# sangminwoo/SVOL

Hardware: AMD Instinct MI355X
Metric: frames/sec (fwd+matcher+bwd), T=32·P=196·d=256 (higher is better)
Workload: dtype bf16

## Files before the change

svol_amd/csrc/common.h:

```cpp
#pragma once
#include <hip/hip_runtime.h>
#include <stdint.h>

#include "../../include/svol_hip.h"

typedef __bf16 bf16_t;
typedef __attribute__((ext_vector_type(8))) __bf16 bf16x8;
typedef __attribute__((ext_vector_type(4))) __bf16 bf16x4;
typedef __attribute__((ext_vector_type(2))) __bf16 bf16x2;
typedef _Float16 f16_t;
typedef __attribute__((ext_vector_type(8))) _Float16 f16x8;
typedef __attribute__((ext_vector_type(4))) _Float16 f16x4;
typedef __attribute__((ext_vector_type(2))) _Float16 f16x2;
typedef __attribute__((ext_vector_type(4))) float f32x4;
typedef __attribute__((ext_vector_type(16))) float f32x16;

#ifdef SVOL_H16_FP16
typedef f16_t h16_t;
typedef f16x8 h16x8;
typedef f16x4 h16x4;
typedef f16x2 h16x2;
#define SVOL_MFMA_16x16x32_H16 __builtin_amdgcn_mfma_f32_16x16x32_f16
#define SVOL_MFMA_32x32x16_H16 __builtin_amdgcn_mfma_f32_32x32x16_f16
#define SVOL_DS_READ_TR16_H16 svol_ds_read_tr16_f16
// ... 93 lines not shown
    DetScratch& operator=(const DetScratch&) = delete;
};
#ifdef __HIPCC__
namespace {
__global__ __launch_bounds__(256) void det_fold_kernel(const float* __restrict__ part, int parts, int64_t pstride, float* __restrict__ dst,
                                                       int64_t n, int64_t bpart, int64_t bdst) {
    const int64_t j = (int64_t)blockIdx.x * 256 + threadIdx.x;
    if (j >= n) return;
    const float* q = part + (int64_t)blockIdx.y * bpart + j;
    float* d = dst + (int64_t)blockIdx.y * bdst + j;
    float acc = *d;
    for (int i = 0; i < parts; ++i) acc += q[(int64_t)i * pstride];
    *d = acc;
}
inline void det_fold(const float* part, int parts, int64_t pstride, float* dst, int64_t n, hipStream_t s, int batches = 1, int64_t bpart = 0,
                     int64_t bdst = 0) {
    if (!dst || n <= 0 || parts <= 0) return;
    hipLaunchKernelGGL(det_fold_kernel, dim3((unsigned)((n + 255) / 256), (unsigned)batches), dim3(256), 0, s, part, parts, pstride, dst, n,
                       bpart, bdst);
}
}
#endif

struct HalfPair { unsigned lo, hi; };
__device__ __forceinline__ HalfPair swap_halves(unsigned x) {
    unsigned y = x;
    asm volatile("" : "+v"(y));
    const auto sw = __builtin_amdgcn_permlane32_swap(x, y, false, false);
    return HalfPair{sw[0], sw[1]};
}

__device__ __forceinline__ float to_f32(float x) { return x; }
__device__ __forceinline__ float to_f32(bf16_t x) { return (float)x; }
__device__ __forceinline__ float to_f32(f16_t x) { return (float)x; }
template <typename T> __device__ __forceinline__ T from_f32(float x);
template <> __device__ __forceinline__ float from_f32<float>(float x) { return x; }
template <> __device__ __forceinline__ bf16_t from_f32<bf16_t>(float x) { return (bf16_t)x; }
template <> __device__ __forceinline__ f16_t from_f32<f16_t>(float x) { return (f16_t)x; }

template <typename T> struct Vec4;
template <> struct Vec4<float> {
    f32x4 v;
    __device__ __forceinline__ void load(const float* p) { v = *reinterpret_cast<const f32x4*>(p); }
    __device__ __forceinline__ void store(float* p) const { *reinterpret_cast<f32x4*>(p) = v; }
    __device__ __forceinline__ float get(int i) const { return v[i]; }
    __device__ __forceinline__ void set(int i, float x) { v[i] = x; }
// ... 113 lines not shown
```

svol_amd/csrc/gate.hip:

```cpp
#include <cstdlib>

#include "common.h"

namespace {

constexpr int GP = 4;
constexpr int GH = 8;
constexpr int GHMAX = 32;

__device__ __forceinline__ void store_head_sums(const float (&part)[GH], float* __restrict__ scores, int b, int l, int L, int H, int lane,
                                                int h0 = 0) {
    const bool b0 = lane & 1, b1 = lane & 2;
    float h4[4], h2[2];
#pragma unroll
    for (int i = 0; i < 4; ++i) {
        const float send = b0 ? part[i] : part[4 + i], keep = b0 ? part[4 + i] : part[i];
        h4[i] = keep + dpp_f32<0xB1>(send);
    }
#pragma unroll
    for (int i = 0; i < 2; ++i) {
        const float send = b1 ? h4[i] : h4[2 + i], keep = b1 ? h4[2 + i] : h4[i];
        h2[i] = keep + dpp_f32<0x4E>(send);
    }
#pragma unroll
    for (int i = 0; i < 2; ++i) {
        float v = h2[i];
        v += dpp_f32<0x124>(v);
        v += dpp_f32<0x128>(v);
        const HalfPair r16 = swap_rows16(__builtin_bit_cast(unsigned, v));
        v = __builtin_bit_cast(float, r16.lo) + __builtin_bit_cast(float, r16.hi);
        const HalfPair r32 = swap_halves(__builtin_bit_cast(unsigned, v));
        h2[i] = __builtin_bit_cast(float, r32.lo) + __builtin_bit_cast(float, r32.hi);
    }
    if (lane < 4) {
        const int hh0 = h0 + 4 * (lane & 1) + 2 * (lane >> 1);
        if (hh0 < H) scores[((int64_t)b * H + hh0) * L + l] = h2[0];
        if (hh0 + 1 < H) scores[((int64_t)b * H + hh0 + 1) * L + l] = h2[1];
    }
}

template <typename T, int NP, bool WIDE = false>
__global__ __launch_bounds__(256) void gate_scores_kernel(const float* __restrict__ x, const T* __restrict__ pos,
                                                          const float* __restrict__ u, float* __restrict__ scores, int L,
                                                          int D, int H, int rpw, int hbase) {
    const int lane = threadIdx.x & 63, wave = threadIdx.x >> 6;
    const int b = blockIdx.y;
    const int l0 = (blockIdx.x * 4 + wave) * rpw;
    const int h0 = WIDE ? hbase : 0;
    float ur[GH][NP][4];
#pragma unroll
    for (int hh = 0; hh < GH; ++hh)
#pragma unroll
        for (int j = 0; j < NP; ++j) {
            const int c = (lane + 64 * j) * 4;
#pragma unroll
            for (int e = 0; e < 4; ++e) ur[hh][j][e] = (h0 + hh < H && c < D) ? u[((int64_t)b * H + h0 + hh) * D + c + e] : 0.f;
        }
    const int lend = min(l0 + rpw, L);
    Vec4<float> xv[NP], nxv[NP];
    Vec4<T> pv[NP], npv[NP];
    auto fetch = [&](int l, Vec4<float> (&xr)[NP], Vec4<T> (&pr)[NP]) {
        const int64_t row = (int64_t)b * L + l;
#pragma unroll
        for (int j = 0; j < NP; ++j) {
            const int c = (lane + 64 * j) * 4;
            if (c < D) {
                xr[j].load(x + row * D + c);
                pr[j].load(pos + row * D + c);
            }
        }
    };
    if (l0 < lend) fetch(l0, xv, pv);
    for (int l = l0; l < lend; ++l) {
        if (l + 1 < lend) fetch(l + 1, nxv, npv);
        float part[GH];
#pragma unroll
        for (int hh = 0; hh < GH; ++hh) part[hh] = 0.f;
#pragma unroll
        for (int j = 0; j < NP; ++j) {
            const int c = (lane + 64 * j) * 4;
            if (c < D) {
#pragma unroll
                for (int e = 0; e < 4; ++e) {
                    const float t = xv[j].get(e) + pv[j].get(e);
#pragma unroll
                    for (int hh = 0; hh < GH; ++hh) part[hh] += t * ur[hh][j][e];
                }
            }
        }
        store_head_sums(part, scores, b, l, L, H, lane, h0);
#pragma unroll
        for (int j = 0; j < NP; ++j) { xv[j] = nxv[j]; pv[j] = npv[j]; }
    }
}

__global__ __launch_bounds__(256) void gate_stats_kernel(const float* __restrict__ scores, float* __restrict__ mx_out,
                                                         float* __restrict__ sm_out, int L) {
    __shared__ float red[4];
    const int bh = blockIdx.x, tid = threadIdx.x, lane = tid & 63, wave = tid >> 6;
    const float* s = scores + (int64_t)bh * L;
    float m = -INFINITY;
    for (int l = tid; l < L; l += 256) m = fmaxf(m, s[l]);
    m = wave_max(m);
    if (lane == 0) red[wave] = m;
    __syncthreads();
    m = fmaxf(fmaxf(red[0], red[1]), fmaxf(red[2], red[3]));
    __syncthreads();
    float acc = 0.f;
    for (int l = tid; l < L; l += 256) acc += __expf(s[l] - m);
    acc = wave_sum(acc);
    if (lane == 0) red[wave] = acc;
    __syncthreads();
    if (tid == 0) {
        mx_out[bh] = m;
        sm_out[bh] = red[0] + red[1] + red[2] + red[3];
    }
// ... 171 lines not shown
        }
    }
    __syncthreads();
    float part[GH];
#pragma unroll
    for (int hh = 0; hh < GH; ++hh) part[hh] = 0.f;
#pragma unroll
    for (int j = 0; j < NP; ++j) {
        const int c = (lane + 64 * j) * 4;
        if (c < D) {
            f32x4 ur[GH];
#pragma unroll
            for (int hh = 0; hh < GH; ++hh) ur[hh] = *reinterpret_cast<const f32x4*>(su + hh * D + c);
#pragma unroll
            for (int e = 0; e < 4; ++e) {
#pragma unroll
                for (int hh = 0; hh < GH; ++hh) part[hh] += tp[j][e] * ur[hh][e];
            }
        }
    }
    store_head_sums(part, scores, b, l, L, H, lane);
}

template <typename T, int NP>
__global__ __launch_bounds__(256) void gate_bwd_ln_kernel(const float* __restrict__ dy32, const T* __restrict__ dy,
                                                          const T* __restrict__ dy2, const float* __restrict__ x,
                                                          const float* __restrict__ a_in,
                                                          const float* __restrict__ gamma, const float* __restrict__ mean,
                                                          const float* __restrict__ rstd, float* __restrict__ dx,
                                                          float* __restrict__ da, float* __restrict__ dgamma,
                                                          float* __restrict__ dbeta, const float* __restrict__ scores,
                                                          const float* __restrict__ mx, const float* __restrict__ sm,
                                                          float* __restrict__ cc, int L, int H, int64_t M, int D, int rpw,
                                                          float* __restrict__ det_cc, float* __restrict__ det_gb) {
    const int lane = threadIdx.x & 63;
    const int64_t r0 = ((int64_t)blockIdx.x * 4 + (threadIdx.x >> 6)) * rpw;
    const int64_t rend = (r0 + rpw < M) ? r0 + rpw : M;
    float dg[NP][4], db[NP][4], gm[NP][4];
    int bcur = r0 < rend ? (int)(r0 / L) : 0, lcur = r0 < rend ? (int)(r0 % L) : 0;
    float cacc = 0.f, mxl = 0.f, isl = 0.f;
    if (lane < H && r0 < rend) { mxl = mx[bcur * H + lane]; isl = 1.f / sm[bcur * H + lane]; }
#pragma unroll
    for (int j = 0; j < NP; ++j) {
        const int c = (lane + 64 * j) * 4;
#pragma unroll
        for (int e = 0; e < 4; ++e) { dg[j][e] = 0.f; db[j][e] = 0.f; gm[j][e] = c < D ? gamma[c + e] : 0.f; }
    }
    struct Row { Vec4<float> p32[NP], xv[NP]; Vec4<T> p[NP], p2[NP]; float mu, rs, a, sc; };
    auto fetch = [&](int64_t row, int b, int l, Row& r) {
#pragma unroll
        for (int j = 0; j < NP; ++j) {
            const int c = (lane + 64 * j) * 4;
            if (c < D) {
                if (dy32) r.p32[j].load(dy32 + row * D + c);
                if (dy) r.p[j].load(dy + row * D + c);
                if (dy2) r.p2[j].load(dy2 + row * D + c);
                r.xv[j].load(x + row * D + c);
            }
        }
        r.mu = mean[row]; r.rs = rstd[row]; r.a = a_in[row];
        r.sc = lane < H ? scores[((int64_t)b * H + lane) * L + l] : 0.f;
    };
    Row cur, nxt;
    if (r0 < rend) fetch(r0, bcur, lcur, cur);
    for (int64_t row = r0; row < rend; ++row) {
        int bn = bcur, ln = lcur + 1;
        if (ln == L) { ln = 0; ++bn; }
        if (row + 1 < rend) fetch(row + 1, bn, ln, nxt);
        const float mu = cur.mu, rs = cur.rs, a = cur.a;
        float g[NP][4], xh[NP][4];
        float s1 = 0.f, s2 = 0.f;
#pragma unroll
        for (int j = 0; j < NP; ++j) {
            const int c = (lane + 64 * j) * 4;
            if (c < D) {
#pragma unroll
                for (int e = 0; e < 4; ++e) {
                    const float d = (dy32 ? cur.p32[j].get(e) : 0.f) + (dy ? cur.p[j].get(e) : 0.f) + (dy2 ? cur.p2[j].get(e) : 0.f);
                    const float hv = (cur.xv[j].get(e) * (1.f + a) - mu) * rs;
                    xh[j][e] = hv;
                    dg[j][e] += d * hv;
                    db[j][e] += d;
                    const float gg = d * gm[j][e];
                    g[j][e] = gg;
                    s1 += gg;
                    s2 += gg * hv;
                }
            }
        }
        s1 = wave_sum(s1) / (float)D;
        s2 = wave_sum(s2) / (float)D;
        float dacc = 0.f;
#pragma unroll
        for (int j = 0; j < NP; ++j) {
            const int c = (lane + 64 * j) * 4;
            if (c < D) {
                Vec4<float> o;
#pragma unroll
                for (int e = 0; e < 4; ++e) {
                    const float ds = rs * (g[j][e] - s1 - xh[j][e] * s2);
                    dacc += ds * cur.xv[j].get(e);
                    o.set(e, ds * (1.f + a));
                }
                o.store(dx + row * D + c);
            }
        }
        dacc = wave_sum(dacc);
        if (lane == 0) da[row] = dacc;
        cacc += __expf(cur.sc - mxl) * isl * dacc;
        if (bn != bcur || row + 1 == rend) {
            if (lane < H) {
                if (det_cc) det_cc[(((int64_t)blockIdx.x * 4 + (threadIdx.x >> 6)) * (M / L) + bcur) * H + lane] = cacc / (float)H;
                else atomicAdd(cc + bcur * H + lane, cacc / (float)H);
                cacc = 0.f;
                if (row + 1 < rend) { mxl = mx[bn * H + lane]; isl = 1.f / sm[bn * H + lane]; }
            }
        }
        bcur = bn;
        lcur = ln;
        cur = nxt;
    }
    __shared__ float red[2][NP * 256];
    const int wave = threadIdx.x >> 6;
    for (int w = 0; w < 4; ++w) {
        if (wave == w) {
#pragma unroll
            for (int j = 0; j < NP; ++j) {
                const int c = (lane + 64 * j) * 4;
                if (c < D) {
#pragma unroll
                    for (int e = 0; e < 4; ++e) {
                        if (w == 0) { red[0][c + e] = dg[j][e]; red[1][c + e] = db[j][e]; }
                        else { red[0][c + e] += dg[j][e]; red[1][c + e] += db[j][e]; }
                    }
                }
            }
        }
        __syncthreads();
    }
    if (det_gb) {
        float* row = det_gb + (int64_t)blockIdx.x * 2 * D;
        for (int c = threadIdx.x; c < D; c += 256) { row[c] = red[0][c]; row[D + c] = red[1][c]; }
        return;
    }
    for (int c = threadIdx.x; c < D; c += 256) {
        atomicAdd(dgamma + c, red[0][c]);
        atomicAdd(dbeta + c, red[1][c]);
    }
}

template <typename T, int NP, bool WIDE = false>
__global__ __launch_bounds__(256) void gate_bwd_apply_kernel(const float* __restrict__ x, const T* __restrict__ pos,
                                                             const float* __restrict__ u, const float* __restrict__ scores,
                                                             const float* __restrict__ mx, const float* __restrict__ sm,
                                                             const float* __restrict__ da, const float* __restrict__ cc,
                                                             float* __restrict__ dx, float* __restrict__ du, int L, int D,
                                                             int H, int rpw, float* __restrict__ det_du, int hbase) {
    const int lane = threadIdx.x & 63, wave = threadIdx.x >> 6;
    const int b = blockIdx.y;
    const int l0 = (blockIdx.x * 4 + wave) * rpw;
    const int h0 = WIDE ? hbase : 0;
    float ur[GH][NP][4], dur[GH][NP][4];
#pragma unroll
    for (int hh = 0; hh < GH; ++hh)
#pragma unroll
        for (int j = 0; j < NP; ++j) {
            const int c = (lane + 64 * j) * 4;
#pragma unroll
            for (int e = 0; e < 4; ++e) {
                ur[hh][j][e] = (h0 + hh < H && c < D) ? u[((int64_t)b * H + h0 + hh) * D + c + e] : 0.f;
                dur[hh][j][e] = 0.f;
            }
        }
    const int lend = min(l0 + rpw, L);
    Vec4<float> xv[NP], dv[NP], nxv[NP], ndv[NP];
    Vec4<T> pv[NP], npv[NP];
    float mxr[GH], isr[GH], ccr[GH], sc[GH], nsc[GH], dar = 0.f, ndar = 0.f;
#pragma unroll
    for (int hh = 0; hh < GH; ++hh) {
        mxr[hh] = h0 + hh < H ? mx[b * H + h0 + hh] : 0.f;
        isr[hh] = h0 + hh < H ? 1.f / sm[b * H + h0 + hh] : 0.f;
        ccr[hh] = h0 + hh < H ? cc[b * H + h0 + hh] : 0.f;
        sc[hh] = nsc[hh] = 0.f;
    }
    auto fetch = [&](int l, Vec4<float> (&xr)[NP], Vec4<T> (&pr)[NP], Vec4<float> (&dr)[NP], float (&sr)[GH], float& dr1) {
        const int64_t row = (int64_t)b * L + l;
#pragma unroll
        for (int j = 0; j < NP; ++j) {
            const int c = (lane + 64 * j) * 4;
            if (c < D) {
                xr[j].load(x + row * D + c);
                pr[j].load(pos + row * D + c);
                dr[j].load(dx + row * D + c);
            }
        }
#pragma unroll
        for (int hh = 0; hh < GH; ++hh)
            if (h0 + hh < H) sr[hh] = scores[((int64_t)b * H + h0 + hh) * L + l];
        dr1 = da[row];
    };
    if (l0 < lend) fetch(l0, xv, pv, dv, sc, dar);
    for (int l = l0; l < lend; ++l) {
        const int64_t row = (int64_t)b * L + l;
        if (l + 1 < lend) fetch(l + 1, nxv, npv, ndv, nsc, ndar);
        float ds[GH];
        const float dal = dar / (float)H;
#pragma unroll
        for (int hh = 0; hh < GH; ++hh) {
            if (h0 + hh < H) {
                const float pp = __expf(sc[hh] - mxr[hh]) * isr[hh];
                ds[hh] = pp * (dal - ccr[hh]);
            } else ds[hh] = 0.f;
        }
#pragma unroll
        for (int j = 0; j < NP; ++j) {
            const int c = (lane + 64 * j) * 4;
            if (c < D) {
#pragma unroll
                for (int e = 0; e < 4; ++e) {
                    const float t = xv[j].get(e) + pv[j].get(e);
                    float add = 0.f;
#pragma unroll
                    for (int hh = 0; hh < GH; ++hh) {
                        add += ds[hh] * ur[hh][j][e];
                        dur[hh][j][e] += ds[hh] * t;
                    }
                    dv[j].set(e, dv[j].get(e) + add);
                }
                dv[j].store(dx + row * D + c);
            }
        }
#pragma unroll
        for (int j = 0; j < NP; ++j) { xv[j] = nxv[j]; pv[j] = npv[j]; dv[j] = ndv[j]; }
#pragma unroll
        for (int hh = 0; hh < GH; ++hh) sc[hh] = nsc[hh];
        dar = ndar;
    }
    __shared__ float red[GH * NP * 256];
    for (int w = 0; w < 4; ++w) {
        if (wave == w) {
#pragma unroll
            for (int hh = 0; hh < GH; ++hh)
#pragma unroll
                for (int j = 0; j < NP; ++j) {
                    const int c = (lane + 64 * j) * 4;
#pragma unroll
                    for (int e = 0; e < 4; ++e) {
                        float* r = red + hh * NP * 256 + c + e;
                        if (w == 0) *r = dur[hh][j][e];
                        else *r += dur[hh][j][e];
                    }
                }
        }
        __syncthreads();
    }
    for (int i = threadIdx.x; i < GH * NP * 256; i += 256) {
        const int hh = i / (NP * 256), c = i % (NP * 256);
        if (h0 + hh < H && c < D) {
            if (det_du) det_du[(((int64_t)b * gridDim.x + blockIdx.x) * H + h0 + hh) * D + c] = red[i];
            else atomicAdd(du + ((int64_t)b * H + h0 + hh) * D + c, red[i]);
// ... 161 lines not shown
}

}

extern "C" {

static int gate_fwd_impl(const float* x32, const void* pos, const float* u, const float* gamma, const float* beta, float* y32,
                         void* y, void* ypos, float* a, float* mean, float* rstd, float* ws, int64_t B, int64_t L, int64_t D, int64_t H,
                         int dtype, void* stream, bool scored) {
    if (!x32 || !pos || !u || !gamma || !beta || (!y && !y32) || !a || !mean || !rstd || !ws) return SVOL_E_INVALID;
    if (!aligned16(gamma) || !aligned16(beta)) return SVOL_E_INVALID;
    if (B <= 0 || L <= 0 || D <= 0 || H <= 0) return SVOL_E_INVALID;
    if (D % 4 || D > GP * 256 || H > (scored ? GH : GHMAX) || B > 65535 || L > (1 << 24)) return SVOL_E_UNSUPPORTED;
    if (!svol_is16(dtype) && dtype != SVOL_F32) return SVOL_E_INVALID;
    hipStream_t s = reinterpret_cast<hipStream_t>(stream);
    const int np_ = D <= 256 ? 1 : (D <= 512 ? 2 : 4);
    float* scores = ws;
    float* mx = ws + B * H * L;
    float* sm = mx + B * H;
    const int rpw = rows_per_wave(L, gate_waves(0) / B + 1);
    dim3 g1((unsigned)((L + 4 * rpw - 1) / (4 * rpw)), (unsigned)B);
    const int64_t M = B * L;
    const unsigned g3 = (unsigned)((M + 3) / 4);
#define SVOL_GATE_SC(TT, N, W, H0) hipLaunchKernelGGL((gate_scores_kernel<TT, N, W>), g1, dim3(256), 0, s, x32, (const TT*)pos, u, scores, (int)L, (int)D, (int)H, rpw, H0)
#define SVOL_GATE_AP(TT, N, W, H0) hipLaunchKernelGGL((gate_apply_kernel<TT, N, W>), dim3(g3), dim3(256), 0, s, x32, (const TT*)pos, scores, mx, sm, gamma, beta, y32, (TT*)y, (TT*)ypos, a, mean, rstd, (int)L, (int)D, (int)H, M)
#define SVOL_GATE_NP(LAUNCH, TT, W, H0)                                                                                     \
    do {                                                                                                                    \
        if (np_ == 1) LAUNCH(TT, 1, W, H0);                                                                                 \
        else if (np_ == 2) LAUNCH(TT, 2, W, H0);                                                                            \
        else LAUNCH(TT, 4, W, H0);                                                                                          \
    } while (0)
#define SVOL_GATE_FWD(TT)                                                                                                   \
    do {                                                                                                                    \
        if (scored) { }                                                                                                      \
        else if (H <= GH) SVOL_GATE_NP(SVOL_GATE_SC, TT, false, 0);                                                         \
        else for (int h0 = 0; h0 < (int)H; h0 += GH) SVOL_GATE_NP(SVOL_GATE_SC, TT, true, h0);                              \
        hipLaunchKernelGGL(gate_stats_kernel, dim3((unsigned)(B * H)), dim3(256), 0, s, scores, mx, sm, (int)L);            \
        if (H <= GH) SVOL_GATE_NP(SVOL_GATE_AP, TT, false, 0);                                                              \
        else SVOL_GATE_NP(SVOL_GATE_AP, TT, true, 0);                                                                       \
    } while (0)
    if (dtype == SVOL_BF16) SVOL_GATE_FWD(bf16_t);
    else if (dtype == SVOL_F16) SVOL_GATE_FWD(f16_t);
    else SVOL_GATE_FWD(float);
#undef SVOL_GATE_FWD
#undef SVOL_GATE_SC
#undef SVOL_GATE_AP
    SVOL_CHECK_LAUNCH();
    return SVOL_OK;
}

int svol_gate_fwd(const float* x32, const void* pos, const float* u, const float* gamma, const float* beta, float* y32,
                  void* y, void* ypos, float* a, float* mean, float* rstd, float* ws, int64_t B, int64_t L, int64_t D, int64_t H,
                  int dtype, void* stream) {
    return gate_fwd_impl(x32, pos, u, gamma, beta, y32, y, ypos, a, mean, rstd, ws, B, L, D, H, dtype, stream, false);
}

int svol_gate_fwd_scored(const float* x32, const void* pos, const float* u, const float* gamma, const float* beta, float* y32,
                         void* y, void* ypos, float* a, float* mean, float* rstd, float* ws, int64_t B, int64_t L, int64_t D,
                         int64_t H, int dtype, void* stream) {
// ... 32 lines not shown
    if (B <= 0 || L <= 0 || D <= 0 || H <= 0) return SVOL_E_INVALID;
    if (D % 4 || D > GP * 256 || H > GHMAX || B > 65535 || L > (1 << 24)) return SVOL_E_UNSUPPORTED;
    if (!svol_is16(dtype) && dtype != SVOL_F32) return SVOL_E_INVALID;
    hipStream_t s = reinterpret_cast<hipStream_t>(stream);
    const int np_ = D <= 256 ? 1 : (D <= 512 ? 2 : 4);
    const float* scores = ws;
    const float* mx = ws + B * H * L;
    const float* sm = mx + B * H;
    float* da = ws2;
    float* cc = ws2 + B * L;
    const int64_t M = B * L;
    const int rpw1 = rows_per_wave(M, gate_waves(1));
    const unsigned g1 = (unsigned)(((M + rpw1 - 1) / rpw1 + 3) / 4);
    const int rpw3 = rows_per_wave(L, gate_waves(2) / B + 1);
    dim3 g3((unsigned)((L + 4 * rpw3 - 1) / (4 * rpw3)), (unsigned)B);
    if (hipMemsetAsync(cc, 0, sizeof(float) * (size_t)(B * H), s) != hipSuccess) return SVOL_E_LAUNCH;
    const bool det_mode = svol_deterministic();
    const size_t n_cc = (size_t)g1 * 4 * (size_t)(B * H), n_gb = (size_t)g1 * 2 * (size_t)D, n_du = (size_t)B * g3.x * (size_t)(H * D);
    DetScratch det(det_mode ? n_cc + n_gb + n_du : 0, s, true);
    if (det_mode && !det.p) return SVOL_E_LAUNCH;
    float* det_cc = det_mode ? det.p : nullptr;
    float* det_gb = det_mode ? det.p + n_cc : nullptr;
    float* det_du = det_mode ? det.p + n_cc + n_gb : nullptr;
#define SVOL_GATE_LN(TT, N, W, H0) hipLaunchKernelGGL((gate_bwd_ln_kernel<TT, N>), dim3(g1), dim3(256), 0, s, dy32, (const TT*)dy, (const TT*)dy2, x32, a, gamma, mean, rstd, dx32, da, dgamma, dbeta, scores, mx, sm, cc, (int)L, (int)H, M, (int)D, rpw1, det_cc, det_gb)
#define SVOL_GATE_BA(TT, N, W, H0) hipLaunchKernelGGL((gate_bwd_apply_kernel<TT, N, W>), g3, dim3(256), 0, s, x32, (const TT*)pos, u, scores, mx, sm, da, cc, dx32, du, (int)L, (int)D, (int)H, rpw3, det_du, H0)
#define SVOL_GATE_BWD(TT)                                                                                                   \
    do {                                                                                                                    \
        SVOL_GATE_NP(SVOL_GATE_LN, TT, false, 0);                                                                           \
        if (det_mode) {                                                                                                     \
            det_fold(det_cc, (int)(g1 * 4), B * H, cc, B * H, s);                                                           \
            det_fold(det_gb, (int)g1, 2 * D, dgamma, D, s);                                                                 \
            det_fold(det_gb + D, (int)g1, 2 * D, dbeta, D, s);                                                              \
        }                                                                                                                   \
        if (H <= GH) SVOL_GATE_NP(SVOL_GATE_BA, TT, false, 0);                                                              \
        else for (int h0 = 0; h0 < (int)H; h0 += GH) SVOL_GATE_NP(SVOL_GATE_BA, TT, true, h0);                              \
    } while (0)
    if (dtype == SVOL_BF16) SVOL_GATE_BWD(bf16_t);
    else if (dtype == SVOL_F16) SVOL_GATE_BWD(f16_t);
    else SVOL_GATE_BWD(float);
#undef SVOL_GATE_BWD
#undef SVOL_GATE_LN
#undef SVOL_GATE_BA
#undef SVOL_GATE_NP
    if (det_mode) det_fold(det_du, (int)g3.x, H * D, du, H * D, s, (int)B, (int64_t)g3.x * H * D, H * D);
    SVOL_CHECK_LAUNCH();
    return SVOL_OK;
}

int svol_gate_vectors_fwd(const float* skch, const float* W_in, const float* b_in, float* q_out, float* u_out, int64_t B, int64_t D,
                          int64_t H, void* stream) {
    if (!skch || !W_in || !b_in || !q_out || !u_out || B <= 0 || D <= 0 || H <= 0) return SVOL_E_INVALID;
    if (D % 4 || D > GP * 256 || H > GHMAX || D % H || B > 65535) return SVOL_E_UNSUPPORTED;
    if (!aligned16(W_in)) return SVOL_E_INVALID;
    hipLaunchKernelGGL(gate_vec_fwd_kernel, dim3((unsigned)H, (unsigned)B), dim3(256), 0, reinterpret_cast<hipStream_t>(stream), skch,
                       W_in, b_in, q_out, u_out, (int)D, (int)H);
    SVOL_CHECK_LAUNCH();
    return SVOL_OK;
}

int svol_gate_vectors_bwd(const float* du, const float* skch, const float* W_in, const float* q, float* dq_ws, float* dskch,
                          float* dW_in, float* db_in, int64_t B, int64_t D, int64_t H, void* stream) {
    if (!du || !skch || !W_in || !q || !dq_ws || !dW_in || !db_in || B <= 0 || D <= 0 || H <= 0) return SVOL_E_INVALID;
    if (D % 4 || D > GP * 256 || H > GHMAX || D % H || B > 65535) return SVOL_E_UNSUPPORTED;
    if (!aligned16(W_in)) return SVOL_E_INVALID;
    hipStream_t s = reinterpret_cast<hipStream_t>(stream);
    hipLaunchKernelGGL(gate_vec_bwd_a_kernel, dim3((unsigned)H, (unsigned)B), dim3(256), 0, s, du, W_in, dq_ws, (int)D, (int)H);
// ... 42 lines not shown
```

svol_amd/csrc/norm.hip:

```cpp
#include "common.h"

namespace {

constexpr int LN_MAX_PASSES = 4;

template <typename T, typename TX, int NP>
__global__ __launch_bounds__(256) void ln_fwd_kernel(const TX* __restrict__ x, const float* __restrict__ gamma,
                                                     const float* __restrict__ beta, float* __restrict__ y32,
                                                     T* __restrict__ y, T* __restrict__ ypos, const T* __restrict__ pos,
                                                     int64_t pos_rows, float* __restrict__ mean, float* __restrict__ rstd,
                                                     int64_t M, int D, float p, float inv_keep, uint64_t seed0,
                                                     const int64_t* __restrict__ soff) {
    const uint64_t seed = seed0 + (soff ? ((uint64_t)soff[0] << 8) : 0ull);
    const int lane = threadIdx.x & 63;
    const int64_t row = (int64_t)blockIdx.x * 4 + (threadIdx.x >> 6);
    if (row >= M) return;
    const TX* xr = x + row * D;
    float v[NP][4];
    float s = 0.f;
    const T* pr = pos ? pos + (row % pos_rows) * D : nullptr;
    Vec4<TX> t[NP];
    Vec4<T> pv[NP];
    Vec4<float> gv[NP], bv[NP];
#pragma unroll
// ... 28 lines not shown
    const float rs = rsqrtf(wave_sum(q) / (float)D + 1e-5f);
    if (lane == 0) { mean[row] = mu; rstd[row] = rs; }
#pragma unroll
    for (int j = 0; j < NP; ++j) {
        const int c = (lane + 64 * j) * 4;
        if (c < D) {
            Vec4<T> o, op;
            Vec4<float> o32;
#pragma unroll
            for (int e = 0; e < 4; ++e) {
                float r = (v[j][e] - mu) * rs * gv[j].get(e) + bv[j].get(e);
                if (p > 0.f) r *= dropout_scale(seed, (uint64_t)row, (uint32_t)(c + e), p, inv_keep);
                o.set(e, r);
                o32.set(e, r);
                if (pr) op.set(e, r + pv[j].get(e));
            }
            if (y32) o32.store(y32 + row * D + c);
            if (y) o.store(y + row * D + c);
            if (ypos) op.store(ypos + row * D + c);
        }
    }
}

template <typename T, typename TX, int NP>
__global__ __launch_bounds__(256) void ln_bwd_kernel(const float* __restrict__ dy32, const T* __restrict__ dy,
                                                     const T* __restrict__ dy2, const TX* __restrict__ x,
                                                     const float* __restrict__ gamma, const float* __restrict__ mean,
                                                     const float* __restrict__ rstd, float* __restrict__ dx32,
                                                     T* __restrict__ dx, float* __restrict__ dgamma,
                                                     float* __restrict__ dbeta, float* __restrict__ dxsum, int64_t M, int D,
                                                     float p, float inv_keep, uint64_t seed0, const int64_t* __restrict__ soff, int rows_per_wave,
                                                     float* __restrict__ det_part) {
    const uint64_t seed = seed0 + (soff ? ((uint64_t)soff[0] << 8) : 0ull);
    const int lane = threadIdx.x & 63;
    const int64_t wave_id = (int64_t)blockIdx.x * 4 + (threadIdx.x >> 6);
    const int64_t r0 = wave_id * rows_per_wave;
    float dg[NP][4], db[NP][4], dxs[NP][4], gm[NP][4];
#pragma unroll
    for (int j = 0; j < NP; ++j) {
        const int c = (lane + 64 * j) * 4;
#pragma unroll
        for (int e = 0; e < 4; ++e) { dg[j][e] = 0.f; db[j][e] = 0.f; dxs[j][e] = 0.f; gm[j][e] = c < D ? gamma[c + e] : 0.f; }
    }
    struct Row { Vec4<float> a32[NP]; Vec4<T> a[NP], b[NP]; Vec4<TX> xv[NP]; float mu, rs; };
    auto fetch = [&](int64_t row, Row& r) {
#pragma unroll
        for (int j = 0; j < NP; ++j) {
            const int c = (lane + 64 * j) * 4;
            if (c < D) {
                if (dy32) r.a32[j].load(dy32 + row * D + c);
                if (dy) r.a[j].load(dy + row * D + c);
                if (dy2) r.b[j].load(dy2 + row * D + c);
                r.xv[j].load(x + row * D + c);
            }
        }
        r.mu = mean[row];
        r.rs = rstd[row];
    };
    const int64_t rend = (r0 + rows_per_wave < M) ? r0 + rows_per_wave : M;
    Row cur, nxt;
    if (r0 < rend) fetch(r0, cur);
    for (int64_t row = r0; row < rend; ++row) {
        if (row + 1 < rend) fetch(row + 1, nxt);
        const float mu = cur.mu, rs = cur.rs;
        float g[NP][4], xh[NP][4];
        float s1 = 0.f, s2 = 0.f;
#pragma unroll
        for (int j = 0; j < NP; ++j) {
            const int c = (lane + 64 * j) * 4;
            if (c < D) {
#pragma unroll
                for (int e = 0; e < 4; ++e) {
                    float d = (dy32 ? cur.a32[j].get(e) : 0.f) + (dy ? cur.a[j].get(e) : 0.f) + (dy2 ? cur.b[j].get(e) : 0.f);
                    if (p > 0.f) d *= dropout_scale(seed, (uint64_t)row, (uint32_t)(c + e), p, inv_keep);
                    const float h = (cur.xv[j].get(e) - mu) * rs;
                    xh[j][e] = h;
                    dg[j][e] += d * h;
                    db[j][e] += d;
                    const float gg = d * gm[j][e];
                    g[j][e] = gg;
                    s1 += gg;
                    s2 += gg * h;
                }
            }
        }
        s1 = wave_sum(s1) / (float)D;
        s2 = wave_sum(s2) / (float)D;
#pragma unroll
        for (int j = 0; j < NP; ++j) {
            const int c = (lane + 64 * j) * 4;
            if (c < D) {
                Vec4<T> o;
                Vec4<float> o32;
#pragma unroll
                for (int e = 0; e < 4; ++e) {
                    const float r = rs * (g[j][e] - s1 - xh[j][e] * s2);
                    dxs[j][e] += r;
                    o.set(e, r);
                    o32.set(e, r);
                }
                if (dx32) o32.store(dx32 + row * D + c);
                if (dx) o.store(dx + row * D + c);
            }
        }
        cur = nxt;
    }
    __shared__ float red[3][NP * 256];
    const int wave = threadIdx.x >> 6;
    for (int w = 0; w < 4; ++w) {
        if (wave == w) {
#pragma unroll
            for (int j = 0; j < NP; ++j) {
                const int c = (lane + 64 * j) * 4;
                if (c < D) {
#pragma unroll
                    for (int e = 0; e < 4; ++e) {
                        if (w == 0) { red[0][c + e] = dg[j][e]; red[1][c + e] = db[j][e]; red[2][c + e] = dxs[j][e]; }
                        else { red[0][c + e] += dg[j][e]; red[1][c + e] += db[j][e]; red[2][c + e] += dxs[j][e]; }
                    }
                }
            }
        }
        __syncthreads();
    }
    if (det_part) {
        float* row = det_part + (int64_t)blockIdx.x * 3 * D;
        for (int c = threadIdx.x; c < D; c += 256) { row[c] = red[0][c]; row[D + c] = red[1][c]; row[2 * D + c] = red[2][c]; }
        return;
    }
// ... 123 lines not shown
    SVOL_CHECK_LAUNCH();
    return SVOL_OK;
}

int svol_layernorm_bwd(const float* dy32, const void* dy, const void* dy2, const void* x, int x_f32, const float* gamma,
                       const float* mean, const float* rstd, float* dx32, void* dx, float* dgamma, float* dbeta,
                       float* dx_colsum, int64_t M, int64_t D, float dropout_p, uint64_t seed, const int64_t* seed_offset_dev,
                       int dtype, void* stream) {
    if ((!dy32 && !dy && !dy2) || !x || !gamma || !mean || !rstd || (!dx && !dx32) || !dgamma || !dbeta || M < 0 || D <= 0)
        return SVOL_E_INVALID;
    if (D % 4 || D > LN_MAX_PASSES * 256) return SVOL_E_UNSUPPORTED;
    if (dropout_p < 0.f || dropout_p >= 1.f) return SVOL_E_INVALID;
    if (!svol_is16(dtype) && dtype != SVOL_F32) return SVOL_E_INVALID;
    if (M == 0) return SVOL_OK;
    const float inv_keep = 1.f / (1.f - dropout_p);
    int64_t rpw = (M + 2047) / 2048;
    if (rpw < 1) rpw = 1;
    const int64_t waves = (M + rpw - 1) / rpw;
    const unsigned grid = (unsigned)((waves + 3) / 4);
    hipStream_t s = reinterpret_cast<hipStream_t>(stream);
    const bool det_mode = svol_deterministic();
    DetScratch det(det_mode ? (size_t)grid * 3 * (size_t)D : 0, s);
    if (det_mode && !det.p) return SVOL_E_LAUNCH;
#define SVOL_LNB(TT, TXX, NPP)                                                                                                      \
    hipLaunchKernelGGL((ln_bwd_kernel<TT, TXX, NPP>), dim3(grid), dim3(256), 0, s, dy32, (const TT*)dy, (const TT*)dy2, (const TXX*)x, \
                       gamma, mean, rstd, dx32, (TT*)dx, dgamma, dbeta, dx_colsum, M, (int)D, dropout_p, inv_keep, seed,              \
                       seed_offset_dev, (int)rpw, det.p)
#define SVOL_LNB_NP(TT, TXX)                  \
    do {                                      \
        if (D <= 256) SVOL_LNB(TT, TXX, 1);   \
        else if (D <= 512) SVOL_LNB(TT, TXX, 2); \
        else SVOL_LNB(TT, TXX, 4);            \
    } while (0)
    if (dtype == SVOL_BF16 && x_f32) SVOL_LNB_NP(bf16_t, float);
    else if (dtype == SVOL_BF16) SVOL_LNB_NP(bf16_t, bf16_t);
    else if (dtype == SVOL_F16 && x_f32) SVOL_LNB_NP(f16_t, float);
    else if (dtype == SVOL_F16) SVOL_LNB_NP(f16_t, f16_t);
    else SVOL_LNB_NP(float, float);
#undef SVOL_LNB_NP
#undef SVOL_LNB
    if (det_mode) {
        det_fold(det.p, (int)grid, 3 * D, dgamma, D, s);
        det_fold(det.p + D, (int)grid, 3 * D, dbeta, D, s);
        det_fold(det.p + 2 * D, (int)grid, 3 * D, dx_colsum, D, s);
    }
    SVOL_CHECK_LAUNCH();
    return SVOL_OK;
}

int svol_dropout_sd(const void* x, void* y, int64_t n, int64_t row_len, float p, uint64_t seed, const int64_t* seed_step_dev, int dtype,
                    void* stream) {
    if (!x || !y || n < 0 || row_len <= 0 || row_len > 0xffffffffll || !(p >= 0.f && p < 1.f)) return SVOL_E_INVALID;
    if (n == 0) return SVOL_OK;
    const float inv = 1.f / (1.f - p);
    int64_t g = (n + 1023) / 1024;
// ... 48 lines not shown
```

Measured before the change: 14980.

## Add templated ring-buffer row prefetch to gate and layernorm backward row loops

Replaces the single next-row double buffer in the gate scores, gate backward LN/apply and layernorm backward kernels with a generic ring of PF prefetched rows. Loads become unconditional by clamping columns and substituting a dummy source for null pointers, which removes branches and keeps more loads in flight. Depth is chosen at runtime from an environment variable and defaults to 2, so by default the pipeline depth matches the old code apart from the branch-free loads and an FMA change. Deeper settings raise register pressure and may reduce occupancy.

```diff
diff --git a/svol_amd/csrc/common.h b/svol_amd/csrc/common.h
--- a/svol_amd/csrc/common.h
+++ b/svol_amd/csrc/common.h
@@ -139,6 +139,42 @@
 }
 #endif
 
+constexpr int ROWLOOP_DEPTH_SHIPPED = 2;
+template <int PF, typename Fetch, typename Body>
+__host__ __device__ __forceinline__ void row_ring(int64_t r0, int64_t rend, Fetch&& fetch, Body&& body) {
+    if (r0 >= rend) return;
+    const int64_t last = rend - 1;
+#pragma unroll
+    for (int s = 0; s < PF; ++s) fetch(r0 + s < last ? r0 + s : last, s);
+    for (int64_t base = r0; base < rend; base += PF) {
+#pragma unroll
+        for (int s = 0; s < PF; ++s) {
+            const int64_t row = base + s;
+            if (row >= rend) return;
+            body(row, s);
+            fetch(row + PF < last ? row + PF : last, s);
+        }
+    }
+}
+__host__ __device__ __forceinline__ int rowloop_col(int c, int D) { return c < D ? c : D - 4; }
+template <typename T> struct RowSrc { const T* p; int64_t ld; };
+template <typename T>
+__host__ __device__ __forceinline__ RowSrc<T> rowloop_src(const T* p, int64_t ld, const float* spare) {
+    return p ? RowSrc<T>{p, ld} : RowSrc<T>{reinterpret_cast<const T*>(spare), 0};
+}
+static inline int svol_rowloop_depth() {
+    static const int depth = [] {
+        const char* e = getenv("SVOL_ROWLOOP_DEPTH");
+        const int v = e ? atoi(e) : ROWLOOP_DEPTH_SHIPPED;
+        return v >= 8 ? 8 : (v >= 4 ? 4 : 2);
+    }();
+    return depth;
+}
+constexpr int rowloop_slots(int depth, int np, int cap = 8) {
+    const int d = depth < cap ? depth : cap;
+    return np == 1 ? d : (np == 2 && d >= 4 && cap >= 8 ? 4 : 2);
+}
+
 struct HalfPair { unsigned lo, hi; };
 __device__ __forceinline__ HalfPair swap_halves(unsigned x) {
     unsigned y = x;
diff --git a/svol_amd/csrc/gate.hip b/svol_amd/csrc/gate.hip
--- a/svol_amd/csrc/gate.hip
+++ b/svol_amd/csrc/gate.hip
@@ -6,6 +6,8 @@
 
 constexpr int GP = 4;
 constexpr int GH = 8;
+constexpr int GATE_AP_SLOTS = 4;
+template <typename T> constexpr int gate_ln_slots() { return sizeof(T) == 4 ? 4 : 8; }
 constexpr int GHMAX = 32;
 
 __device__ __forceinline__ void store_head_sums(const float (&part)[GH], float* __restrict__ scores, int b, int l, int L, int H, int lane,
@@ -39,7 +41,7 @@
     }
 }
 
-template <typename T, int NP, bool WIDE = false>
+template <typename T, int NP, int PF, bool WIDE = false>
 __global__ __launch_bounds__(256) void gate_scores_kernel(const float* __restrict__ x, const T* __restrict__ pos,
                                                           const float* __restrict__ u, float* __restrict__ scores, int L,
                                                           int D, int H, int rpw, int hbase) {
@@ -57,41 +59,38 @@
             for (int e = 0; e < 4; ++e) ur[hh][j][e] = (h0 + hh < H && c < D) ? u[((int64_t)b * H + h0 + hh) * D + c + e] : 0.f;
         }
     const int lend = min(l0 + rpw, L);
-    Vec4<float> xv[NP], nxv[NP];
-    Vec4<T> pv[NP], npv[NP];
-    auto fetch = [&](int l, Vec4<float> (&xr)[NP], Vec4<T> (&pr)[NP]) {
+    struct Row { Vec4<float> xv[NP]; Vec4<T> pv[NP]; };
+    Row ring[PF];
+    auto fetch = [&](int64_t l, int slot) __attribute__((always_inline)) {
+        Row& r = ring[slot];
         const int64_t row = (int64_t)b * L + l;
+#pragma unroll
+        for (int j = 0; j < NP; ++j) {
+            const int c = rowloop_col((lane + 64 * j) * 4, D);
+            r.xv[j].load(x + row * D + c);
+            r.pv[j].load(pos + row * D + c);
+        }
+    };
+    auto body = [&](int64_t l, int slot) __attribute__((always_inline)) {
+        const Row& cur = ring[slot];
+        float part[GH];
+#pragma unroll
+        for (int hh = 0; hh < GH; ++hh) part[hh] = 0.f;
 #pragma unroll
         for (int j = 0; j < NP; ++j) {
             const int c = (lane + 64 * j) * 4;
             if (c < D) {
-                xr[j].load(x + row * D + c);
-                pr[j].load(pos + row * D + c);
-            }
-        }
-    };
-    if (l0 < lend) fetch(l0, xv, pv);
-    for (int l = l0; l < lend; ++l) {
-        if (l + 1 < lend) fetch(l + 1, nxv, npv);
-        float part[GH];
-#pragma unroll
-        for (int hh = 0; hh < GH; ++hh) part[hh] = 0.f;
-#pragma unroll
-        for (int j = 0; j < NP; ++j) {
-            const int c = (lane + 64 * j) * 4;
-            if (c < D) {
 #pragma unroll
                 for (int e = 0; e < 4; ++e) {
-                    const float t = xv[j].get(e) + pv[j].get(e);
+                    const float t = cur.xv[j].get(e) + cur.pv[j].get(e);
 #pragma unroll
                     for (int hh = 0; hh < GH; ++hh) part[hh] += t * ur[hh][j][e];
                 }
             }
         }
-        store_head_sums(part, scores, b, l, L, H, lane, h0);
-#pragma unroll
-        for (int j = 0; j < NP; ++j) { xv[j] = nxv[j]; pv[j] = npv[j]; }
-    }
+        store_head_sums(part, scores, b, (int)l, L, H, lane, h0);
+    };
+    row_ring<PF>(l0, lend, fetch, body);
 }
 
 __global__ __launch_bounds__(256) void gate_stats_kernel(const float* __restrict__ scores, float* __restrict__ mx_out,
@@ -309,7 +308,7 @@
     store_head_sums(part, scores, b, l, L, H, lane);
 }
 
-template <typename T, int NP>
+template <typename T, int NP, int PF>
 __global__ __launch_bounds__(256) void gate_bwd_ln_kernel(const float* __restrict__ dy32, const T* __restrict__ dy,
                                                           const T* __restrict__ dy2, const float* __restrict__ x,
                                                           const float* __restrict__ a_in,
@@ -334,26 +333,34 @@
         for (int e = 0; e < 4; ++e) { dg[j][e] = 0.f; db[j][e] = 0.f; gm[j][e] = c < D ? gamma[c + e] : 0.f; }
     }
     struct Row { Vec4<float> p32[NP], xv[NP]; Vec4<T> p[NP], p2[NP]; float mu, rs, a, sc; };
-    auto fetch = [&](int64_t row, int b, int l, Row& r) {
+    Row ring[PF];
+    int bf = bcur, lf = lcur;
+    int64_t rf = r0;
+    const RowSrc<float> q32 = rowloop_src(dy32, D, gamma);
+    const RowSrc<T> qa = rowloop_src(dy, D, gamma), qb = rowloop_src(dy2, D, gamma);
+    const int hl = lane < H ? lane : H - 1;
+    auto fetch = [&](int64_t row, int slot) __attribute__((always_inline)) {
+        Row& r = ring[slot];
+        lf += row != rf ? 1 : 0;
+        rf = row;
+        const bool wrap = lf == L;
+        lf = wrap ? 0 : lf;
+        bf += wrap ? 1 : 0;
 #pragma unroll
         for (int j = 0; j < NP; ++j) {
-            const int c = (lane + 64 * j) * 4;
-            if (c < D) {
-                if (dy32) r.p32[j].load(dy32 + row * D + c);
-                if (dy) r.p[j].load(dy + row * D + c);
-                if (dy2) r.p2[j].load(dy2 + row * D + c);
-                r.xv[j].load(x + row * D + c);
-            }
+            const int c = rowloop_col((lane + 64 * j) * 4, D);
+            r.p32[j].load(q32.p + row * q32.ld + c);
+            r.p[j].load(qa.p + row * qa.ld + c);
+            r.p2[j].load(qb.p + row * qb.ld + c);
+            r.xv[j].load(x + row * D + c);
         }
         r.mu = mean[row]; r.rs = rstd[row]; r.a = a_in[row];
-        r.sc = lane < H ? scores[((int64_t)b * H + lane) * L + l] : 0.f;
+        r.sc = scores[((int64_t)bf * H + hl) * L + lf];
     };
-    Row cur, nxt;
-    if (r0 < rend) fetch(r0, bcur, lcur, cur);
-    for (int64_t row = r0; row < rend; ++row) {
+    auto body = [&](int64_t row, int slot) __attribute__((always_inline)) {
+        const Row& cur = ring[slot];
         int bn = bcur, ln = lcur + 1;
         if (ln == L) { ln = 0; ++bn; }
-        if (row + 1 < rend) fetch(row + 1, bn, ln, nxt);
         const float mu = cur.mu, rs = cur.rs, a = cur.a;
         float g[NP][4], xh[NP][4];
         float s1 = 0.f, s2 = 0.f;
@@ -366,7 +373,7 @@
                     const float d = (dy32 ? cur.p32[j].get(e) : 0.f) + (dy ? cur.p[j].get(e) : 0.f) + (dy2 ? cur.p2[j].get(e) : 0.f);
                     const float hv = (cur.xv[j].get(e) * (1.f + a) - mu) * rs;
                     xh[j][e] = hv;
-                    dg[j][e] += d * hv;
+                    dg[j][e] = __builtin_fmaf(d, hv, dg[j][e]);
                     db[j][e] += d;
                     const float gg = d * gm[j][e];
                     g[j][e] = gg;
@@ -405,8 +412,8 @@
         }
         bcur = bn;
         lcur = ln;
-        cur = nxt;
-    }
+    };
+    row_ring<PF>(r0, rend, fetch, body);
     __shared__ float red[2][NP * 256];
     const int wave = threadIdx.x >> 6;
     for (int w = 0; w < 4; ++w) {
@@ -436,7 +443,7 @@
     }
 }
 
-template <typename T, int NP, bool WIDE = false>
+template <typename T, int NP, int PF, bool WIDE = false>
 __global__ __launch_bounds__(256) void gate_bwd_apply_kernel(const float* __restrict__ x, const T* __restrict__ pos,
                                                              const float* __restrict__ u, const float* __restrict__ scores,
                                                              const float* __restrict__ mx, const float* __restrict__ sm,
@@ -460,69 +467,61 @@
             }
         }
     const int lend = min(l0 + rpw, L);
-    Vec4<float> xv[NP], dv[NP], nxv[NP], ndv[NP];
-    Vec4<T> pv[NP], npv[NP];
-    float mxr[GH], isr[GH], ccr[GH], sc[GH], nsc[GH], dar = 0.f, ndar = 0.f;
+    float mxr[GH], isr[GH], ccr[GH];
 #pragma unroll
     for (int hh = 0; hh < GH; ++hh) {
         mxr[hh] = h0 + hh < H ? mx[b * H + h0 + hh] : 0.f;
         isr[hh] = h0 + hh < H ? 1.f / sm[b * H + h0 + hh] : 0.f;
         ccr[hh] = h0 + hh < H ? cc[b * H + h0 + hh] : 0.f;
-        sc[hh] = nsc[hh] = 0.f;
-    }
-    auto fetch = [&](int l, Vec4<float> (&xr)[NP], Vec4<T> (&pr)[NP], Vec4<float> (&dr)[NP], float (&sr)[GH], float& dr1) {
+    }
+    struct Row { Vec4<float> xv[NP], dv[NP]; Vec4<T> pv[NP]; float sc[GH], da; };
+    Row ring[PF];
+    auto fetch = [&](int64_t l, int slot) __attribute__((always_inline)) {
+        Row& r = ring[slot];
         const int64_t row = (int64_t)b * L + l;
+#pragma unroll
+        for (int j = 0; j < NP; ++j) {
+            const int c = rowloop_col((lane + 64 * j) * 4, D);
+            r.xv[j].load(x + row * D + c);
+            r.pv[j].load(pos + row * D + c);
+            r.dv[j].load(dx + row * D + c);
+        }
+#pragma unroll
+        for (int hh = 0; hh < GH; ++hh) r.sc[hh] = scores[((int64_t)b * H + min(h0 + hh, H - 1)) * L + l];
+        r.da = da[row];
+    };
+    auto body = [&](int64_t l, int slot) __attribute__((always_inline)) {
+        Row& cur = ring[slot];
+        const int64_t row = (int64_t)b * L + l;
+        float ds[GH];
+        const float dal = cur.da / (float)H;
+#pragma unroll
+        for (int hh = 0; hh < GH; ++hh) {
+            if (h0 + hh < H) {
+                const float pp = __expf(cur.sc[hh] - mxr[hh]) * isr[hh];
+                ds[hh] = pp * (dal - ccr[hh]);
+            } else ds[hh] = 0.f;
+        }
 #pragma unroll
         for (int j = 0; j < NP; ++j) {
             const int c = (lane + 64 * j) * 4;
             if (c < D) {
-                xr[j].load(x + row * D + c);
-                pr[j].load(pos + row * D + c);
-                dr[j].load(dx + row * D + c);
-            }
-        }
-#pragma unroll
-        for (int hh = 0; hh < GH; ++hh)
-            if (h0 + hh < H) sr[hh] = scores[((int64_t)b * H + h0 + hh) * L + l];
-        dr1 = da[row];
-    };
-    if (l0 < lend) fetch(l0, xv, pv, dv, sc, dar);
-    for (int l = l0; l < lend; ++l) {
-        const int64_t row = (int64_t)b * L + l;
-        if (l + 1 < lend) fetch(l + 1, nxv, npv, ndv, nsc, ndar);
-        float ds[GH];
-        const float dal = dar / (float)H;
-#pragma unroll
-        for (int hh = 0; hh < GH; ++hh) {
-            if (h0 + hh < H) {
-                const float pp = __expf(sc[hh] - mxr[hh]) * isr[hh];
-                ds[hh] = pp * (dal - ccr[hh]);
-            } else ds[hh] = 0.f;
-        }
-#pragma unroll
-        for (int j = 0; j < NP; ++j) {
-            const int c = (lane + 64 * j) * 4;
-            if (c < D) {
 #pragma unroll
                 for (int e = 0; e < 4; ++e) {
-                    const float t = xv[j].get(e) + pv[j].get(e);
+                    const float t = cur.xv[j].get(e) + cur.pv[j].get(e);
                     float add = 0.f;
 #pragma unroll
                     for (int hh = 0; hh < GH; ++hh) {
                         add += ds[hh] * ur[hh][j][e];
                         dur[hh][j][e] += ds[hh] * t;
                     }
-                    dv[j].set(e, dv[j].get(e) + add);
+                    cur.dv[j].set(e, cur.dv[j].get(e) + add);
                 }
-                dv[j].store(dx + row * D + c);
-            }
-        }
-#pragma unroll
-        for (int j = 0; j < NP; ++j) { xv[j] = nxv[j]; pv[j] = npv[j]; dv[j] = ndv[j]; }
-#pragma unroll
-        for (int hh = 0; hh < GH; ++hh) sc[hh] = nsc[hh];
-        dar = ndar;
-    }
+                cur.dv[j].store(dx + row * D + c);
+            }
+        }
+    };
+    row_ring<PF>(l0, lend, fetch, body);
     __shared__ float red[GH * NP * 256];
     for (int w = 0; w < 4; ++w) {
         if (wave == w) {
@@ -730,7 +729,7 @@
     dim3 g1((unsigned)((L + 4 * rpw - 1) / (4 * rpw)), (unsigned)B);
     const int64_t M = B * L;
     const unsigned g3 = (unsigned)((M + 3) / 4);
-#define SVOL_GATE_SC(TT, N, W, H0) hipLaunchKernelGGL((gate_scores_kernel<TT, N, W>), g1, dim3(256), 0, s, x32, (const TT*)pos, u, scores, (int)L, (int)D, (int)H, rpw, H0)
+#define SVOL_GATE_SC(TT, N, PFF, W, H0) hipLaunchKernelGGL((gate_scores_kernel<TT, N, PFF, W>), g1, dim3(256), 0, s, x32, (const TT*)pos, u, scores, (int)L, (int)D, (int)H, rpw, H0)
 #define SVOL_GATE_AP(TT, N, W, H0) hipLaunchKernelGGL((gate_apply_kernel<TT, N, W>), dim3(g3), dim3(256), 0, s, x32, (const TT*)pos, scores, mx, sm, gamma, beta, y32, (TT*)y, (TT*)ypos, a, mean, rstd, (int)L, (int)D, (int)H, M)
 #define SVOL_GATE_NP(LAUNCH, TT, W, H0)                                                                                     \
     do {                                                                                                                    \
@@ -738,11 +737,23 @@
         else if (np_ == 2) LAUNCH(TT, 2, W, H0);                                                                            \
         else LAUNCH(TT, 4, W, H0);                                                                                          \
     } while (0)
+#define SVOL_GATE_NP_PF(LAUNCH, TT, W, H0, CAP, CAP2)                                                                       \
+    do {                                                                                                                    \
+        const int pf_ = rowloop_slots(svol_rowloop_depth(), np_, np_ == 2 ? 2 * CAP2 : CAP);                                \
+        if (np_ == 1) {                                                                                                     \
+            if (pf_ == 8) LAUNCH(TT, 1, (CAP < 8 ? CAP : 8), W, H0);                                                        \
+            else if (pf_ == 4) LAUNCH(TT, 1, 4, W, H0);                                                                     \
+            else LAUNCH(TT, 1, 2, W, H0);                                                                                   \
+        } else if (np_ == 2) {                                                                                              \
+            if (pf_ == 4) LAUNCH(TT, 2, (CAP2 < 4 ? 2 : 4), W, H0);                                                         \
+            else LAUNCH(TT, 2, 2, W, H0);                                                                                   \
+        } else LAUNCH(TT, 4, 2, W, H0);                                                                                     \
+    } while (0)
 #define SVOL_GATE_FWD(TT)                                                                                                   \
     do {                                                                                                                    \
         if (scored) { }                                                                                                      \
-        else if (H <= GH) SVOL_GATE_NP(SVOL_GATE_SC, TT, false, 0);                                                         \
-        else for (int h0 = 0; h0 < (int)H; h0 += GH) SVOL_GATE_NP(SVOL_GATE_SC, TT, true, h0);                              \
+        else if (H <= GH) SVOL_GATE_NP_PF(SVOL_GATE_SC, TT, false, 0, 8, 4);                                                   \
+        else for (int h0 = 0; h0 < (int)H; h0 += GH) SVOL_GATE_NP_PF(SVOL_GATE_SC, TT, true, h0, 8, 4);                        \
         hipLaunchKernelGGL(gate_stats_kernel, dim3((unsigned)(B * H)), dim3(256), 0, s, scores, mx, sm, (int)L);            \
         if (H <= GH) SVOL_GATE_NP(SVOL_GATE_AP, TT, false, 0);                                                              \
         else SVOL_GATE_NP(SVOL_GATE_AP, TT, true, 0);                                                                       \
@@ -821,18 +832,18 @@
     float* det_cc = det_mode ? det.p : nullptr;
     float* det_gb = det_mode ? det.p + n_cc : nullptr;
     float* det_du = det_mode ? det.p + n_cc + n_gb : nullptr;
-#define SVOL_GATE_LN(TT, N, W, H0) hipLaunchKernelGGL((gate_bwd_ln_kernel<TT, N>), dim3(g1), dim3(256), 0, s, dy32, (const TT*)dy, (const TT*)dy2, x32, a, gamma, mean, rstd, dx32, da, dgamma, dbeta, scores, mx, sm, cc, (int)L, (int)H, M, (int)D, rpw1, det_cc, det_gb)
-#define SVOL_GATE_BA(TT, N, W, H0) hipLaunchKernelGGL((gate_bwd_apply_kernel<TT, N, W>), g3, dim3(256), 0, s, x32, (const TT*)pos, u, scores, mx, sm, da, cc, dx32, du, (int)L, (int)D, (int)H, rpw3, det_du, H0)
+#define SVOL_GATE_LN(TT, N, PFF, W, H0) hipLaunchKernelGGL((gate_bwd_ln_kernel<TT, N, PFF>), dim3(g1), dim3(256), 0, s, dy32, (const TT*)dy, (const TT*)dy2, x32, a, gamma, mean, rstd, dx32, da, dgamma, dbeta, scores, mx, sm, cc, (int)L, (int)H, M, (int)D, rpw1, det_cc, det_gb)
+#define SVOL_GATE_BA(TT, N, PFF, W, H0) hipLaunchKernelGGL((gate_bwd_apply_kernel<TT, N, PFF, W>), g3, dim3(256), 0, s, x32, (const TT*)pos, u, scores, mx, sm, da, cc, dx32, du, (int)L, (int)D, (int)H, rpw3, det_du, H0)
 #define SVOL_GATE_BWD(TT)                                                                                                   \
     do {                                                                                                                    \
-        SVOL_GATE_NP(SVOL_GATE_LN, TT, false, 0);                                                                           \
+        SVOL_GATE_NP_PF(SVOL_GATE_LN, TT, false, 0, gate_ln_slots<TT>(), 2);                                                   \
         if (det_mode) {                                                                                                     \
             det_fold(det_cc, (int)(g1 * 4), B * H, cc, B * H, s);                                                           \
             det_fold(det_gb, (int)g1, 2 * D, dgamma, D, s);                                                                 \
             det_fold(det_gb + D, (int)g1, 2 * D, dbeta, D, s);                                                              \
         }                                                                                                                   \
-        if (H <= GH) SVOL_GATE_NP(SVOL_GATE_BA, TT, false, 0);                                                              \
-        else for (int h0 = 0; h0 < (int)H; h0 += GH) SVOL_GATE_NP(SVOL_GATE_BA, TT, true, h0);                              \
+        if (H <= GH) SVOL_GATE_NP_PF(SVOL_GATE_BA, TT, false, 0, GATE_AP_SLOTS, 2);                                            \
+        else for (int h0 = 0; h0 < (int)H; h0 += GH) SVOL_GATE_NP_PF(SVOL_GATE_BA, TT, true, h0, GATE_AP_SLOTS, 2);            \
     } while (0)
     if (dtype == SVOL_BF16) SVOL_GATE_BWD(bf16_t);
     else if (dtype == SVOL_F16) SVOL_GATE_BWD(f16_t);
@@ -841,6 +852,7 @@
 #undef SVOL_GATE_LN
 #undef SVOL_GATE_BA
 #undef SVOL_GATE_NP
+#undef SVOL_GATE_NP_PF
     if (det_mode) det_fold(det_du, (int)g3.x, H * D, du, H * D, s, (int)B, (int64_t)g3.x * H * D, H * D);
     SVOL_CHECK_LAUNCH();
     return SVOL_OK;
diff --git a/svol_amd/csrc/norm.hip b/svol_amd/csrc/norm.hip
--- a/svol_amd/csrc/norm.hip
+++ b/svol_amd/csrc/norm.hip
@@ -74,7 +74,7 @@
     }
 }
 
-template <typename T, typename TX, int NP>
+template <typename T, typename TX, int NP, int PF>
 __global__ __launch_bounds__(256) void ln_bwd_kernel(const float* __restrict__ dy32, const T* __restrict__ dy,
                                                      const T* __restrict__ dy2, const TX* __restrict__ x,
                                                      const float* __restrict__ gamma, const float* __restrict__ mean,
@@ -95,25 +95,25 @@
         for (int e = 0; e < 4; ++e) { dg[j][e] = 0.f; db[j][e] = 0.f; dxs[j][e] = 0.f; gm[j][e] = c < D ? gamma[c + e] : 0.f; }
     }
     struct Row { Vec4<float> a32[NP]; Vec4<T> a[NP], b[NP]; Vec4<TX> xv[NP]; float mu, rs; };
-    auto fetch = [&](int64_t row, Row& r) {
+    Row ring[PF];
+    const RowSrc<float> q32 = rowloop_src(dy32, D, gamma);
+    const RowSrc<T> qa = rowloop_src(dy, D, gamma), qb = rowloop_src(dy2, D, gamma);
+    auto fetch = [&](int64_t row, int slot) __attribute__((always_inline)) {
+        Row& r = ring[slot];
 #pragma unroll
         for (int j = 0; j < NP; ++j) {
-            const int c = (lane + 64 * j) * 4;
-            if (c < D) {
-                if (dy32) r.a32[j].load(dy32 + row * D + c);
-                if (dy) r.a[j].load(dy + row * D + c);
-                if (dy2) r.b[j].load(dy2 + row * D + c);
-                r.xv[j].load(x + row * D + c);
-            }
+            const int c = rowloop_col((lane + 64 * j) * 4, D);
+            r.a32[j].load(q32.p + row * q32.ld + c);
+            r.a[j].load(qa.p + row * qa.ld + c);
+            r.b[j].load(qb.p + row * qb.ld + c);
+            r.xv[j].load(x + row * D + c);
         }
         r.mu = mean[row];
         r.rs = rstd[row];
     };
     const int64_t rend = (r0 + rows_per_wave < M) ? r0 + rows_per_wave : M;
-    Row cur, nxt;
-    if (r0 < rend) fetch(r0, cur);
-    for (int64_t row = r0; row < rend; ++row) {
-        if (row + 1 < rend) fetch(row + 1, nxt);
+    auto body = [&](int64_t row, int slot) __attribute__((always_inline)) {
+        const Row& cur = ring[slot];
         const float mu = cur.mu, rs = cur.rs;
         float g[NP][4], xh[NP][4];
         float s1 = 0.f, s2 = 0.f;
@@ -155,8 +155,8 @@
                 if (dx) o.store(dx + row * D + c);
             }
         }
-        cur = nxt;
-    }
+    };
+    row_ring<PF>(r0, rend, fetch, body);
     __shared__ float red[3][NP * 256];
     const int wave = threadIdx.x >> 6;
     for (int w = 0; w < 4; ++w) {
@@ -326,15 +326,21 @@
     const bool det_mode = svol_deterministic();
     DetScratch det(det_mode ? (size_t)grid * 3 * (size_t)D : 0, s);
     if (det_mode && !det.p) return SVOL_E_LAUNCH;
-#define SVOL_LNB(TT, TXX, NPP)                                                                                                      \
-    hipLaunchKernelGGL((ln_bwd_kernel<TT, TXX, NPP>), dim3(grid), dim3(256), 0, s, dy32, (const TT*)dy, (const TT*)dy2, (const TXX*)x, \
+    const int depth = svol_rowloop_depth();
+#define SVOL_LNB(TT, TXX, NPP, PFF)                                                                                                 \
+    hipLaunchKernelGGL((ln_bwd_kernel<TT, TXX, NPP, PFF>), dim3(grid), dim3(256), 0, s, dy32, (const TT*)dy, (const TT*)dy2, (const TXX*)x, \
                        gamma, mean, rstd, dx32, (TT*)dx, dgamma, dbeta, dx_colsum, M, (int)D, dropout_p, inv_keep, seed,              \
                        seed_offset_dev, (int)rpw, det.p)
-#define SVOL_LNB_NP(TT, TXX)                  \
-    do {                                      \
-        if (D <= 256) SVOL_LNB(TT, TXX, 1);   \
-        else if (D <= 512) SVOL_LNB(TT, TXX, 2); \
-        else SVOL_LNB(TT, TXX, 4);            \
+#define SVOL_LNB_NP(TT, TXX)                                   \
+    do {                                                       \
+        if (D <= 256) {                                        \
+            if (depth == 8) SVOL_LNB(TT, TXX, 1, 8);           \
+            else if (depth == 4) SVOL_LNB(TT, TXX, 1, 4);      \
+            else SVOL_LNB(TT, TXX, 1, 2);                      \
+        } else if (D <= 512) {                                 \
+            if (rowloop_slots(depth, 2) == 4) SVOL_LNB(TT, TXX, 2, 4); \
+            else SVOL_LNB(TT, TXX, 2, 2);                      \
+        } else SVOL_LNB(TT, TXX, 4, 2);                        \
     } while (0)
     if (dtype == SVOL_BF16 && x_f32) SVOL_LNB_NP(bf16_t, float);
     else if (dtype == SVOL_BF16) SVOL_LNB_NP(bf16_t, bf16_t);
```

Measured after the change: 14540. 0.97x the previous value.
